# lnkloveating/MediQuery-RAG

Measured on AMD Instinct MI355X. Metric: queries/s (embed+top-k, k=5, b=256) over 1M×768 corpus; p50 single-query ms, higher is better.
Workload: dtype f32 (exact 3-way bf16 split, fp32 accumulate; exact fp32 top-k)

## Files before the change

include/mq.h:

```cpp
#ifndef MQ_H
#define MQ_H

#include <stdint.h>

#ifdef __cplusplus
extern "C" {
#endif

#define MQ_OK 0
#define MQ_EINVAL -1
#define MQ_ENOMEM -2
#define MQ_EHIP -3
#define MQ_EIO -4
#define MQ_ESTATE -5

#define MQ_DTYPE_F32 0
#define MQ_DTYPE_BF16 1
#define MQ_DTYPE_F32X6 2
#define MQ_DTYPE_F32_SCREEN 3

#define MQ_GELU_ERF 0
#define MQ_GELU_TANH 1
#define MQ_POOL_CLS 0
#define MQ_POOL_MEAN 1
// ... 10 lines not shown
int mq_device_count(void);

int mq_index_create(int device, int dim, int64_t capacity, int dtype, mq_index** out);
int mq_index_destroy(mq_index* ix);
int mq_index_size(const mq_index* ix, int64_t* n_rows);
int mq_index_dim(const mq_index* ix, int* dim);
int mq_index_add(mq_index* ix, const float* rows, int64_t n, int rows_on_device, void* stream);
int mq_index_reset(mq_index* ix);
int mq_index_search(mq_index* ix, const float* queries, int64_t nq, int k,
                    float* out_scores, int64_t* out_ids, int io_on_device, void* stream);
int mq_index_select(mq_index* src, const int64_t* rows, int64_t n, mq_index* dst);
int mq_index_get(mq_index* ix, int64_t row0, int64_t n, float* out, int out_on_device, void* stream);
int mq_index_set_precision(mq_index* ix, int dtype);
int mq_index_set_stream_threshold(mq_index* ix, int max_queries);
int mq_index_set_threshold_scan(mq_index* ix, int enabled);
int mq_index_set_int8_screen(mq_index* ix, int enabled);
int mq_index_set_async_screen(mq_index* ix, int enabled);
int mq_index_rescans(const mq_index* ix, int64_t* rescans, int64_t* remerges);
int mq_index_screen_fallbacks(const mq_index* ix, int64_t* to_direct, int64_t* to_split);
int mq_index_screen_skips(const mq_index* ix, int64_t* bf16_skips, int64_t* int8_skips);
int mq_index_data(mq_index* ix, void** device_rows);
int mq_index_set_timing(mq_index* ix, int enabled);
int mq_index_read_timing(mq_index* ix, float* ms, int n);
#define MQ_MASK_SET 0
#define MQ_MASK_AND 1
#define MQ_MASK_OR 2
#define MQ_MASK_CLEAR 3
int mq_mask_eval(const int32_t* codes, int64_t n, const uint8_t* lut, int n_lut, uint32_t* bits, int mode,
                 void* stream);
int mq_mask_eval_bits(const int32_t* codes, int64_t n, const uint64_t* lut_words, int n_lut, uint32_t* bits,
// ... 200 lines not shown
```

mediquery-rag_amd/csrc/index.hip:

```cpp
#include <algorithm>
#include <cmath>
#include <cstring>
#include <limits>
#include <memory>
#include <vector>

#include <unistd.h>

#include "common.hpp"
#include "gemm_f32.hpp"
#include "thresh.hpp"
#include "topk.hpp"

namespace mq {

__global__ __launch_bounds__(256) void add_rows_kernel(const float* __restrict__ src,
                                                       float* __restrict__ dst, int64_t n,
                                                       int dim) {
  const int lane = threadIdx.x & 63;
  const int64_t row = (int64_t)blockIdx.x * 4 + (threadIdx.x >> 6);
  if (row >= n) return;
  const floatx4* s = reinterpret_cast<const floatx4*>(src + row * dim);
  floatx4* d = reinterpret_cast<floatx4*>(dst + row * dim);
  const int nv = dim >> 2;
// ... 741 lines not shown
  }
  __syncthreads();
  MQ_FIN_TS(6);
  if (tid == 0) {
    const bool cert = ranked && nlive_sh <= kFinLive &&
                      (nl >= k ? tau[q] + e_sh < ek_sh : tau[q] == -INFINITY);
    if (!cert) fail[atomicAdd(n_fail, 1)] = q;
#if MQ_FIN_DBG & 16
    printf("FIN cnt %d nl %d dt %llu %llu %llu %llu %llu %llu\n", cnt, nl, tsx[1] - tsx[0], tsx[2] - tsx[1],
           tsx[3] - tsx[2], tsx[4] - tsx[3], tsx[5] - tsx[4], tsx[6] - tsx[5]);
#endif
  }
#undef MQ_FIN_TS
}

template <int KC, typename IdIn>
__device__ __forceinline__ void merge_threadlists(const float* __restrict__ cs,
                                                  const IdIn* __restrict__ ci, int n_lists,
                                                  int64_t nq, int k_in, int k_out,
                                                  float* __restrict__ out_s,
                                                  int64_t* __restrict__ out_i, int list_kc,
                                                  int* __restrict__ overflow, int64_t q) {
  constexpr int U = 8;
  __shared__ float ws[4 * MQ_MAX_K];
  __shared__ long long wi[4 * MQ_MAX_K];
  __shared__ float kth_s;
  __shared__ long long kth_i;
  const int tid = threadIdx.x, lane = tid & 63, wave = tid >> 6;
  float ls[KC];
  long long li[KC];
// ... 285 lines not shown
  } else {
    const ScanGeom g = scan_geom(nf, SearchNarrow::BM, SearchNarrow::BN, per_cu, num_cus, n_rows);
    if ((int)blockIdx.x >= g.G * g.nqt) return;
    flat_search_block<SearchNarrow, KC>(lds, Qc, nf, C, n_rows, dim, g.G, g.nqt, kl, cand_s, cand_i, blockIdx.x);
  }
}

template <int KC, int SCAN_KC>
__global__ __launch_bounds__(256) void fallback_merge_kernel(const float* __restrict__ cs,
                                                             const int* __restrict__ ci, int num_cus,
                                                             int64_t n_rows, int k, int kl,
                                                             const int* __restrict__ n_fail,
                                                             const int64_t* __restrict__ fail,
                                                             float* __restrict__ os,
                                                             int64_t* __restrict__ oi,
                                                             unsigned long long* __restrict__ total) {
  const int nf = __builtin_amdgcn_readfirstlane(*n_fail);
  const int64_t j = blockIdx.x;
  if (j == 0 && threadIdx.x == 0 && nf > 0) atomicAdd(total, (unsigned long long)nf);
  if (j >= nf) return;
  constexpr int per_cu = SCAN_KC <= 16 ? 2 : 1;
  int n_lists;
  if (nf > kFbNarrowMax) {
    const ScanGeom g = scan_geom(nf, SearchWide::BM, SearchWide::BN, per_cu, num_cus, n_rows);
    n_lists = g.G * SearchWide::WAVES_N * SearchSmem<SearchWide>::LPQ;
  } else {
    const ScanGeom g = scan_geom(nf, SearchNarrow::BM, SearchNarrow::BN, per_cu, num_cus, n_rows);
    n_lists = g.G * SearchNarrow::WAVES_N * SearchSmem<SearchNarrow>::LPQ;
  }
  const int64_t shift = (fail[j] - j) * k;
  merge_select_block<KC, int>(cs, ci, n_lists, nf, kl, k, os + shift, oi + shift, kl, nullptr, j);
}

}
// ... 42 lines not shown
  DevBuf stage, cand_s, cand_i, out_s, out_i;
  DevBuf sel;
  DevBuf rows16;
  int64_t n16 = 0;
  DevBuf stats16;
  DevBuf q16, coarse_s, coarse_i;
  DevBuf fb_cs, fb_ci;
  DevBuf flag;
  DevBuf tier_fail[4], tier_q[4], tier_s[4], tier_i[4];
  int64_t rescans = 0;
  int64_t remerges = 0;
  int64_t screen_fallbacks = 0;
  int64_t screen_passdowns = 0;
  int stream_max_q = 4;
  bool thresh_scan = true;
  DevBuf ts_lmax, ts_tau, ts_count, ts_cs, ts_ci;
  DevBuf i8c_cs, i8c_ci, i8c_count;
  DevBuf msel, mblk;
  DevBuf mres_s, mres_i;
  PinBuf pin;
  DevBuf rows8, scale8, err8, stats8;
  int64_t n8 = 0;
  int64_t masked_gathers = 0;
  bool i8_screen = true;
  double i8_fail_avg = 0.0;
  int i8_skip = 0;
  int64_t i8_skips = 0;
  bool async_screen = true;
  int sync_left = 0;
  DevBuf afb_q, afb_cs, afb_ci, afb_total;
  unsigned long long* afb_host = nullptr;
  hipEvent_t afb_event = nullptr;
  unsigned long long afb_seen = 0;
  double bf_fail_avg = 0.0;
  int bf_skip = 0;
  int64_t bf_skips = 0;
  Timeline tl;
  int precision = MQ_DTYPE_F32;
  std::mutex mu;
};

namespace {

template <class T, int KC>
void launch_search(const mq_index* ix, const float* q, int nq, int k, int G, int nqt,
                   float* cs, int* ci, hipStream_t s) {
// ... 218 lines not shown
  if (rc) return rc;
  const int64_t qpairs = nq * ix->dim / 2;
  hipLaunchKernelGGL(to_bf16_kernel, dim3((unsigned)((qpairs + 255) / 256)), dim3(256), 0, s, q,
                     ix->q16.as<unsigned>(), qpairs);
  MQ_HIP(hipGetLastError());
  return MQ_OK;
}

bool thresh_ok(const mq_index* ix, int64_t nq) {
  const int nch = ix->dim / 64;
  return ix->thresh_scan && nq > 64 && ix->dim % 64 == 0 && (nch == 4 || nch == 8 || nch == 12) &&
         ix->n >= kTsMinRows && ix->n < (1ll << 31);
}

int thresh_topk(mq_index* ix, const float* q16, int64_t nq, int kc, float* os, int64_t* oi,
                hipStream_t s, int tau_rank, int* fail_count, int64_t* fail, const unsigned* mask = nullptr) {
  const size_t n_lists = 2 * (size_t)ix->num_cus;
  int rc = ix->ts_lmax.ensure(n_lists * nq * sizeof(float));
  if (!rc) rc = ix->ts_tau.ensure(nq * sizeof(float));
  if (!rc) rc = ix->ts_count.ensure(nq * sizeof(int));
  if (!rc) rc = ix->ts_cs.ensure((size_t)nq * kTsCap * sizeof(float));
  if (!rc) rc = ix->ts_ci.ensure((size_t)nq * kTsCap * sizeof(int));
  if (rc) return rc;
  ThreshArgs a{q16, (int)nq, ix->rows16.as<unsigned char>(), ix->n, ix->dim, ix->num_cus, kc,
               ix->ts_lmax.as<float>(), ix->ts_tau.as<float>(), ix->ts_count.as<int>(),
               ix->ts_cs.as<float>(), ix->ts_ci.as<int>(), os, oi, tau_rank, fail_count, fail, mask};
  if (ix->tl.used > 4096) ix->tl.drain();
  launch_thresh(a, s, &ix->tl);
  ix->tl.close(s);
  MQ_HIP(hipGetLastError());
  return MQ_OK;
}

int ensure_i8(mq_index* ix, hipStream_t s) {
  int rc = ix->rows8.ensure((size_t)(ix->cap + kI8PadRows) * ix->dim);
  if (!rc) rc = ix->scale8.ensure((size_t)(ix->cap + kI8PadRows) * sizeof(float));
  if (!rc) rc = ix->err8.ensure((size_t)(ix->cap + kI8PadRows) * sizeof(float));
  if (!rc) rc = ix->stats8.ensure(2 * sizeof(unsigned));
  if (rc) return rc;
  if (ix->n8 < ix->n) {
    if (ix->n8 == 0) MQ_HIP(hipMemsetAsync(ix->stats8.p, 0, 2 * sizeof(unsigned), s));
    launch_i8_shadow(ix->rows + ix->n8 * ix->dim, ix->n - ix->n8, ix->dim,
                     ix->rows8.as<unsigned>() + ix->n8 * ix->dim / 4, ix->scale8.as<float>() + ix->n8,
// ... 142 lines not shown
}

template <class T>
void fallback_extent(const mq_index* ix, int64_t nf_lo, int64_t nf_hi, int per_cu, int kl,
                     int64_t* grid, int64_t* cand) {
  for (int64_t nqt = (nf_lo + T::BM - 1) / T::BM; nqt * T::BM < nf_hi + T::BM; ++nqt) {
    const int64_t nf = std::min(nf_hi, nqt * T::BM);
    const ScanGeom g = scan_geom(nf, T::BM, T::BN, per_cu, ix->num_cus, ix->n);
    *grid = std::max<int64_t>(*grid, (int64_t)g.G * g.nqt);
    *cand = std::max<int64_t>(*cand, (int64_t)g.G * T::WAVES_N * SearchSmem<T>::LPQ * nf * kl);
  }
}

template <int KC>
void launch_fallback_scans(mq_index* ix, int64_t nq, int k, const int* nf, const int64_t* fail,
                           float* os, int64_t* oi, int64_t grid, hipStream_t s) {
  const float* qc = ix->afb_q.as<float>();
  float* cs = ix->afb_cs.as<float>();
  int* ci = ix->afb_ci.as<int>();
  hipLaunchKernelGGL((fallback_search_kernel<KC>), dim3((unsigned)grid), dim3(256), 0, s, qc, nf, ix->rows,
                     ix->n, ix->dim, ix->num_cus, k, cs, ci);
  auto* tot = ix->afb_total.as<unsigned long long>();
  const dim3 mgrid((unsigned)nq);
  if (k <= 8)
    hipLaunchKernelGGL((fallback_merge_kernel<8, KC>), mgrid, dim3(256), 0, s, cs, ci, ix->num_cus, ix->n, k, k,
                       nf, fail, os, oi, tot);
  else
    hipLaunchKernelGGL((fallback_merge_kernel<16, KC>), mgrid, dim3(256), 0, s, cs, ci, ix->num_cus, ix->n, k,
                       k, nf, fail, os, oi, tot);
}

constexpr size_t kFbMaxBytes = 256ull << 20;

struct FallbackPlan {
  bool ok = false;
  int64_t grid = 0;
};

int fallback_prepare(mq_index* ix, int64_t nq, int k, FallbackPlan* fp) {
  const int per_cu = 2;
  int64_t grid_n = 0, grid_w = 0, cand = 0;
  fallback_extent<SearchNarrow>(ix, 1, std::min<int64_t>(nq, kFbNarrowMax), per_cu, k, &grid_n, &cand);
  if (nq > kFbNarrowMax) fallback_extent<SearchWide>(ix, kFbNarrowMax + 1, nq, per_cu, k, &grid_w, &cand);
  fp->ok = false;
  if ((size_t)cand * (sizeof(float) + sizeof(int)) + (size_t)nq * ix->dim * sizeof(float) > kFbMaxBytes)
    return MQ_OK;
  int rc = ix->afb_q.ensure((size_t)nq * ix->dim * sizeof(float));
  if (!rc) rc = ix->afb_cs.ensure((size_t)cand * sizeof(float));
  if (!rc) rc = ix->afb_ci.ensure((size_t)cand * sizeof(int));
  if (!rc && !ix->afb_total.p) {
    rc = ix->afb_total.ensure(sizeof(unsigned long long));
    if (!rc) MQ_HIP(hipMemset(ix->afb_total.p, 0, sizeof(unsigned long long)));
  }
  if (rc) return rc;
  if (!ix->afb_host) {
    MQ_HIP(hipHostMalloc((void**)&ix->afb_host, sizeof(unsigned long long), hipHostMallocDefault));
    *ix->afb_host = 0;
  }
  if (!ix->afb_event) MQ_HIP(hipEventCreateWithFlags(&ix->afb_event, hipEventDisableTiming));
  fp->ok = true;
  fp->grid = std::max(grid_n, grid_w);
  return MQ_OK;
}

static_assert(kScreenMaxK <= 16, "fallback_search_kernel<KC> has KC = 8 or 16");
int launch_async_fallback(mq_index* ix, const FallbackPlan& fp, int64_t nq, int k, float* os, int64_t* oi,
                          const int64_t* fail, hipStream_t s) {
  const int* nf = ix->flag.as<int>();
  if (k <= 8)
    launch_fallback_scans<8>(ix, nq, k, nf, fail, os, oi, fp.grid, s);
  else
    launch_fallback_scans<16>(ix, nq, k, nf, fail, os, oi, fp.grid, s);
  MQ_HIP(hipGetLastError());
  MQ_HIP(hipMemcpyAsync(ix->afb_host, ix->afb_total.p, sizeof(unsigned long long), hipMemcpyDeviceToHost, s));
  MQ_HIP(hipEventRecord(ix->afb_event, s));
  return MQ_OK;
}

int search_screened(mq_index* ix, int tier, const float* q, int64_t nq, int k, float* os,
                    int64_t* oi, hipStream_t s) {
  const bool bf = tier == TIER_BF16_STREAM || tier == TIER_BF16;
  const int want = tier == TIER_BF16 || tier == TIER_I8 ? MQ_MAX_K
                   : tier == TIER_BF16_STREAM ? (k + 11 <= 16 ? 16 : std::min(std::max(32, k + 16), MQ_MAX_K))
                   : (k + 3 <= 8 ? 8 : k + 8);
  const int kc = (int)std::min<int64_t>(want, ix->n);
  int rc = bf ? ensure_shadow(ix, s) : MQ_OK;
  if (!rc && tier == TIER_BF16) rc = queries_to_bf16(ix, q, nq, s);
  if (!rc) rc = ix->coarse_s.ensure((size_t)nq * kc * sizeof(float));
  if (!rc) rc = ix->coarse_i.ensure((size_t)nq * kc * sizeof(int64_t));
  if (!rc) rc = ix->flag.ensure(sizeof(int));
  if (!rc) rc = ix->tier_fail[tier].ensure((size_t)nq * sizeof(int64_t));
  if (rc) return rc;
  int64_t* fail = ix->tier_fail[tier].as<int64_t>();
  if (tier == TIER_I8) {
    rc = i8_topk(ix, q, nq, kc, nullptr, nullptr, s, ix->flag.as<int>(), k);
    if (rc) return rc;
    hipLaunchKernelGGL(i8_finish_kernel, dim3((unsigned)nq), dim3(kFinT), 0, s, q, ix->rows, ix->dim,
                       ix->ts_cs.as<float>(), ix->ts_ci.as<int>(), ix->ts_count.as<int>(),
                       i8_lists(ix->num_cus), ix->ts_tau.as<float>(), k, ix->stats8.as<unsigned>(), ix->err8.as<float>(), os, oi, ix->flag.as<int>(), fail);
    ix->tl.close(s);
    MQ_HIP(hipGetLastError());
  } else {
    const int kind = tier == TIER_X6 ? SCAN_X6 : tier == TIER_BF16 ? SCAN_BF16 : SCAN_STREAM16;
    const float* qs = tier == TIER_BF16 ? ix->q16.as<float>() : q;
    rc = kind == SCAN_BF16 ? bf16_candidates(ix, qs, nq, kc, ix->coarse_s.as<float>(), ix->coarse_i.as<int64_t>(), s)
                           : scan_topk(ix, kind, qs, nq, kc, ix->coarse_s.as<float>(), ix->coarse_i.as<int64_t>(), s);
    if (rc) return rc;
    const int mode = tier == TIER_X6 ? VERIFY_X6 : tier == TIER_BF16 ? VERIFY_BF16_Q16 : VERIFY_BF16_Q32;
    const unsigned* stats = bf ? ix->stats16.as<unsigned>() : nullptr;
// ... 3 lines not shown
    if (kc >= ix->n) return MQ_OK;
    FallbackPlan fp;
    if (tier == TIER_BF16) {
      poll_async_fallbacks(ix);
      if (ix->async_screen && ix->sync_left == 0 && k <= kScreenMaxK) {
        rc = fallback_prepare(ix, nq, k, &fp);
        if (rc) return rc;
      }
      if (!fp.ok && ix->sync_left > 0) --ix->sync_left;
    }
    MQ_HIP(hipMemsetAsync(ix->flag.p, 0, sizeof(int), s));
    hipLaunchKernelGGL(screen_verify_kernel, dim3((unsigned)((nq + 3) / 4)), dim3(256), 0, s, q,
                       ix->dim, ix->coarse_s.as<float>(), kc, os, k, nq, mode, stats, ix->flag.as<int>(),
                       fail, fp.ok ? ix->afb_q.as<float>() : nullptr);
    MQ_HIP(hipGetLastError());
    if (fp.ok) return launch_async_fallback(ix, fp, nq, k, os, oi, fail, s);
  }
  int n_fail = 0;
  rc = read_flag(ix, ix->flag.as<int>(), s, &n_fail);
  if (rc) return rc;
  if (tier == TIER_I8) {
    ix->i8_fail_avg = 0.9 * ix->i8_fail_avg + 0.1 * (double)n_fail / (double)nq;
    if (ix->i8_fail_avg > 0.3) {
      ix->i8_skip = 256;
      ix->i8_fail_avg = 0.0;
    }
  } else if (tier == TIER_BF16) {
    ix->bf_fail_avg = 0.75 * ix->bf_fail_avg + 0.25 * (double)n_fail / (double)nq;
    if (ix->bf_fail_avg > kBfSkipShare) {
      ix->bf_skip = kBfSkipSearches;
      ix->bf_fail_avg = 0.0;
// ... 358 lines not shown
  if (!stream_ok(ix)) {
    for (int64_t j = 0; j < nq; ++j) {
      const int rc = search_masked(ix, q + j * ix->dim, k, bits, os + j * k, oi + j * k, s);
      if (rc) return rc;
    }
    return MQ_OK;
  }
  if (!(exact_kind && k <= kScreenMaxK && thresh_ok(ix, nq) && ix->dim <= 1024)) {
    const int rc = masked_stream(ix, q, nq, k, bits, os, oi, s);
    if (rc) return rc;
    MQ_HIP(hipStreamSynchronize(s));
    return MQ_OK;
  }
  const int kc = (int)std::min<int64_t>(MQ_MAX_K, ix->n);
  int rc = ensure_shadow(ix, s);
  if (!rc) rc = queries_to_bf16(ix, q, nq, s);
  if (!rc) rc = ix->coarse_s.ensure((size_t)nq * kc * sizeof(float));
  if (!rc) rc = ix->coarse_i.ensure((size_t)nq * kc * sizeof(int64_t));
  if (!rc) rc = ix->flag.ensure(sizeof(int));
  if (!rc) rc = ix->tier_fail[TIER_BF16].ensure((size_t)nq * sizeof(int64_t));
  if (rc) return rc;
  rc = thresh_topk(ix, ix->q16.as<float>(), nq, kc, ix->coarse_s.as<float>(), ix->coarse_i.as<int64_t>(), s,
                   kTsRank, nullptr, nullptr, bits);
  if (rc) return rc;
  const unsigned* stats = ix->stats16.as<unsigned>();
  hipLaunchKernelGGL(rerank_kernel, dim3((unsigned)nq), dim3(256), 0, s, q, ix->rows, ix->dim,
                     ix->coarse_i.as<int64_t>(), kc, k, os, oi, ix->coarse_s.as<float>(), VERIFY_BF16_Q16, stats);
  MQ_HIP(hipMemsetAsync(ix->flag.p, 0, sizeof(int), s));
  int64_t* fail = ix->tier_fail[TIER_BF16].as<int64_t>();
  hipLaunchKernelGGL(screen_verify_kernel, dim3((unsigned)((nq + 3) / 4)), dim3(256), 0, s, q, ix->dim,
                     ix->coarse_s.as<float>(), kc, os, k, nq, VERIFY_BF16_Q16, stats, ix->flag.as<int>(), fail,
                     nullptr);
  MQ_HIP(hipGetLastError());
  int n_fail = 0;
  rc = read_flag(ix, ix->flag.as<int>(), s, &n_fail);
  if (rc) return rc;
  if (n_fail > 0) {
    ix->masked_gathers += n_fail;
    rc = ix->tier_q[TIER_BF16].ensure((size_t)n_fail * ix->dim * sizeof(float));
    if (!rc) rc = ix->tier_s[TIER_BF16].ensure((size_t)n_fail * k * sizeof(float));
    if (!rc) rc = ix->tier_i[TIER_BF16].ensure((size_t)n_fail * k * sizeof(int64_t));
    if (rc) return rc;
    float* sq = ix->tier_q[TIER_BF16].as<float>();
    hipLaunchKernelGGL(gather_rows_kernel, dim3((unsigned)((n_fail + 3) / 4)), dim3(256), 0, s, q, fail,
                       (int64_t)n_fail, ix->dim, sq);
    MQ_HIP(hipGetLastError());
    rc = masked_stream(ix, sq, n_fail, k, bits, ix->tier_s[TIER_BF16].as<float>(),
                       ix->tier_i[TIER_BF16].as<int64_t>(), s);
// ... 213 lines not shown
  MQ_CHECK_ARG(max_queries >= 0 && max_queries <= 16, "stream threshold must be in [0, 16] (got %d)",
               max_queries);
  std::lock_guard<std::mutex> lk(ix->mu);
  ix->stream_max_q = max_queries;
  return MQ_OK;
}

int mq_index_set_threshold_scan(mq_index* ix, int enabled) {
  clear_error();
  MQ_CHECK_ARG(ix, "NULL index");
  std::lock_guard<std::mutex> lk(ix->mu);
  ix->thresh_scan = enabled != 0;
  return MQ_OK;
}

int mq_index_set_int8_screen(mq_index* ix, int enabled) {
  clear_error();
  MQ_CHECK_ARG(ix, "NULL index");
  std::lock_guard<std::mutex> lk(ix->mu);
  ix->i8_screen = enabled != 0;
  ix->i8_skip = 0;
  ix->i8_fail_avg = 0.0;
  return MQ_OK;
}

int mq_index_screen_fallbacks(const mq_index* cix, int64_t* to_direct, int64_t* to_split) {
  clear_error();
  MQ_CHECK_ARG(cix, "NULL argument");
  mq_index* ix = const_cast<mq_index*>(cix);
  hipEvent_t ev = nullptr;
// ... 246 lines not shown
```

mediquery-rag_amd/csrc/thresh.hip:

```cpp
#include "gemm_f32.hpp"

#ifndef MQ_TS_DBG
#define MQ_TS_DBG 0
#endif
#if MQ_TS_DBG != 0 && !defined(MQ_MEASUREMENT_BUILD)
#error "MQ_TS_DBG computes wrong results: only a measurement build (-DMQ_MEASUREMENT_BUILD) may set it"
#endif
#include "thresh.hpp"
#include "topk.hpp"

namespace mq {

constexpr int kTsWaves = 8;
#ifndef MQ_TS_DMAW
#define MQ_TS_DMAW 4
#endif
constexpr int kTsDmaWaves = MQ_TS_DMAW;
static_assert(kTsDmaWaves == 8 || kTsDmaWaves == 4 || kTsDmaWaves == 2 || kTsDmaWaves == 1, "DMA waves");
constexpr int kTsQ = kTsWaves * 32;
constexpr int kTsBufs = 3;
constexpr int kTsPeriod = 16;
#ifndef MQ_TS_BF_PERIOD
#define MQ_TS_BF_PERIOD 16
#endif
// ... 186 lines not shown
    if (qvalid) lmax[(int64_t)q * (2 * gridDim.x) + blockIdx.x * 2 + h] = mx;
  } else {
    for (int j = lane; j < min(n_surv, kTsWaveSurv); j += 64) {
      const Survivor v = surv[j];
      const int slot = atomicAdd(count + v.q, 1);
      if (slot < kTsCap) {
        cs[(int64_t)v.q * kTsCap + slot] = v.s;
        ci[(int64_t)v.q * kTsCap + slot] = v.row;
      }
    }
  }
}

__global__ __launch_bounds__(256) void bf16_tau_kernel(const float* __restrict__ lmax, int n_lists,
                                                       int nq, int rank, float* __restrict__ tau,
                                                       int* __restrict__ count) {
  const int lane = threadIdx.x & 63;
  const int q = blockIdx.x * 4 + (threadIdx.x >> 6);
  if (q >= nq) return;
  TopList<kTsRank> t;
  t.init();
  for (int l = lane; l < n_lists; l += 64) {
    const float x = lmax[(int64_t)q * n_lists + l];
    if (t.beats_tail(x, l)) t.insert(x, l);
  }
  float kth = -INFINITY;
  for (int r = 0; r < rank; ++r) {
    float bs = t.s[0];
    int bi = t.id[0], bt = lane;
#pragma unroll
    for (int off = 32; off > 0; off >>= 1) {
// ... 10 lines not shown
  }
  if (lane == 0) {
    tau[q] = kth;
    count[q] = 0;
  }
}

__global__ __launch_bounds__(256) void bf16_select_kernel(const float* __restrict__ cs,
                                                          const int* __restrict__ ci,
                                                          const int* __restrict__ count,
                                                          const float* __restrict__ tau, int kc,
                                                          float* __restrict__ out_s,
                                                          int64_t* __restrict__ out_i,
                                                          int* __restrict__ fail_count,
                                                          int64_t* __restrict__ fail) {
  __shared__ float ls[kTsCap], fs[kTsCap], ts[256];
  __shared__ int li[kTsCap], fi[kTsCap], ti[256];
  __shared__ float cut_s;
  __shared__ int cut_i, nf;
  const int64_t q = blockIdx.x;
  const int tid = threadIdx.x;
  const int total = count[q];
  if (fail && tid == 0 && (total > kTsCap || total < kc)) fail[atomicAdd(fail_count, 1)] = q;
  const int cnt = min(total, kTsCap);
  float bs = -INFINITY;
  int bi = -1;
  for (int i = tid; i < cnt; i += 256) {
    const float x = cs[q * kTsCap + i];
    const int xi = ci[q * kTsCap + i];
    ls[i] = x;
    li[i] = xi;
    if (bi == -1 || better(x, (unsigned)xi, bs, (unsigned)bi)) {
      bs = x;
      bi = xi;
    }
  }
  auto rank_out = [&](const float* rs, const int* ri, int m) __attribute__((always_inline)) {
    for (int i = tid; i < m; i += 256) {
      const float x = rs[i];
      const int xi = ri[i];
      int rank = 0;
      for (int j = 0; j < m; ++j) rank += better(rs[j], (unsigned)ri[j], x, (unsigned)xi) ? 1 : 0;
      if (rank < kc) {
        out_s[q * kc + rank] = rank == kc - 1 && total > kTsCap ? INFINITY : x;
        out_i[q * kc + rank] = xi;
      }
    }
  };
  if (cnt <= 256) {
    __syncthreads();
    rank_out(ls, li, cnt);
  } else {
    ts[tid] = bs;
    ti[tid] = bi;
    if (tid == 0) {
      cut_s = -INFINITY;
      cut_i = -1;
      nf = 0;
    }
    __syncthreads();
    int rank = 0;
    for (int j = 0; j < 256; ++j) rank += better(ts[j], (unsigned)ti[j], bs, (unsigned)bi) ? 1 : 0;
    if (rank == kc - 1) {
      cut_s = bs;
      cut_i = bi;
    }
    __syncthreads();
    const float Ts = cut_s;
    const unsigned Ti = (unsigned)cut_i;
    const int lane = tid & 63;
    for (int base = 0; base < cnt; base += 256) {
      const int i = base + tid;
      const bool keep = i < cnt && !better(Ts, Ti, ls[i], (unsigned)li[i]);
      const unsigned long long bal = __ballot(keep);
      int slot0 = 0;
      if (lane == 0 && bal) slot0 = atomicAdd(&nf, __popcll(bal));
      slot0 = __shfl(slot0, 0);
      if (keep) {
        const int slot = slot0 + __builtin_amdgcn_mbcnt_hi((unsigned)(bal >> 32), __builtin_amdgcn_mbcnt_lo((unsigned)bal, 0));
        fs[slot] = ls[i];
        fi[slot] = li[i];
      }
    }
    __syncthreads();
    rank_out(fs, fi, nf);
  }
  for (int i = cnt + tid; i < kc; i += 256) {
    out_s[q * kc + i] = tau[q];
    out_i[q * kc + i] = -1;
  }
}

template <int NCH, bool MASKED>
void launch_nch(const ThreshArgs& a, hipStream_t s, Timeline* tl) {
  const int gy = (a.nq + kTsQ - 1) / kTsQ;
  const int G = gy == 1 ? a.num_cus : std::max(8, a.num_cus / gy / 8 * 8);
  const int64_t n_blocks = (a.n + kTsRows - 1) / kTsRows;
  const uint4* qb = reinterpret_cast<const uint4*>(a.q16);
  tl->mark(s, 0);
  hipLaunchKernelGGL((bf16_thresh_kernel<NCH, TS_MAX, MASKED>), dim3(G, gy), dim3(512), 0, s, qb, a.nq, a.rows,
                     a.n, n_blocks, kTsBfPeriod, a.tau, a.lmax, a.count, a.cs, a.ci, a.mask);
  tl->mark(s, 1);
  hipLaunchKernelGGL(bf16_tau_kernel, dim3((a.nq + 3) / 4), dim3(256), 0, s, a.lmax, 2 * G, a.nq,
                     a.tau_rank, a.tau, a.count);
  tl->mark(s, 0);
  hipLaunchKernelGGL((bf16_thresh_kernel<NCH, TS_APPEND, MASKED>), dim3(G, gy), dim3(512), 0, s, qb, a.nq,
                     a.rows, a.n, n_blocks, 1, a.tau, a.lmax, a.count, a.cs, a.ci, a.mask);
  tl->mark(s, 1);
  hipLaunchKernelGGL(bf16_select_kernel, dim3(a.nq), dim3(256), 0, s, a.cs, a.ci, a.count, a.tau, a.kc,
                     a.out_s, a.out_i, a.fail_count, a.fail);
}

template <bool MASKED>
void launch_dim(const ThreshArgs& a, hipStream_t s, Timeline* tl) {
  switch (a.dim / 64) {
    case 4: launch_nch<4, MASKED>(a, s, tl); break;
    case 8: launch_nch<8, MASKED>(a, s, tl); break;
    default: launch_nch<12, MASKED>(a, s, tl); break;
  }
}

void launch_thresh(const ThreshArgs& a, hipStream_t s, Timeline* tl) {
  if (a.mask)
// ... 482 lines not shown
```

mediquery-rag_amd/csrc/thresh.hpp:

```cpp
#pragma once

#include "common.hpp"

namespace mq {

constexpr int kTsRows = 32;
constexpr int kTsCap = 4096;
constexpr int64_t kTsMinRows = 65536;
constexpr int kTsRank = 8;

struct ThreshArgs {
  const float* q16;
  int nq;
  const unsigned char* rows;
  int64_t n;
  int dim;
  int num_cus;
  int kc;
  float* lmax;
  float* tau;
  int* count;
  float* cs;
  int* ci;
  float* out_s;
  int64_t* out_i;
  int tau_rank;
  int* fail_count;
  int64_t* fail;
  const unsigned* mask = nullptr;
};

void launch_thresh(const ThreshArgs& a, hipStream_t s, Timeline* tl);
hipError_t launch_thresh_append(const ThreshArgs& a, hipStream_t s);

#ifndef MQ_I8_WG
#define MQ_I8_WG 3
#endif
constexpr int kI8WgPerCu = MQ_I8_WG;
constexpr int kI8MaxLists = 1024;
constexpr int kI8PadRows = 16;
constexpr int kI8Seg = 16;
struct ThreshI8Args {
  const float* q;
  int nq;
// ... 9 lines not shown
  int* ci;
  int* zero;
  const unsigned* stats = nullptr;
  int k = 0;
  const unsigned* mask = nullptr;
};
int i8_lists(int num_cus);
void launch_i8_compact(const float* cs, const int* ci, const int* count, int lists, int nq, float* out_cs,
                       int* out_ci, int* out_count, hipStream_t s);
void launch_thresh_i8(const ThreshI8Args& a, hipStream_t s, Timeline* tl);
void launch_select(const float* cs, const int* ci, const int* count, const float* tau, int nq, int kc,
                   float* out_s, int64_t* out_i, hipStream_t s);
void launch_i8_shadow(const float* rows, int64_t n, int dim, unsigned* r8, float* scale, float* err,
                      unsigned* stats, hipStream_t s);

}
```

mediquery-rag_amd/mediquery_hip/_lib.py:

```python
import ctypes
import hashlib
import os

try:
    import torch
except Exception:
    torch = None

LIB_PATH = os.environ.get("MQ_LIB_PATH") or os.path.join(os.path.dirname(os.path.abspath(__file__)),
                                                          "libmqhip.so")

MQ_OK = 0
MQ_DTYPE_F32, MQ_DTYPE_BF16, MQ_DTYPE_F32X6, MQ_DTYPE_F32_SCREEN = 0, 1, 2, 3
MQ_GELU_ERF, MQ_GELU_TANH = 0, 1
MQ_POOL_CLS, MQ_POOL_MEAN = 0, 1
MQ_MAX_K = 64
MQ_RANGE_MAX_HITS = 4096
MQ_HEAD_MAX_LABELS = 8
MQ_JOIN_AUTO, MQ_JOIN_EXACT, MQ_JOIN_SCREEN = 0, 1, 2
MQ_KMEANS_MAX_CLUSTERS = 256
MQ_MASK_SET, MQ_MASK_AND, MQ_MASK_OR, MQ_MASK_CLEAR = 0, 1, 2, 3
MQ_CONTAINS_MAX_BYTES = 256
MQ_CONTAINS_SPAN_BYTES = 16384
MQ_LEX_MAX_TERMS = 128
# ... 42 lines not shown
    "mq_build_source_hash": (ctypes.c_char_p, []),
    "mq_device_count": (_I, []),
    "mq_index_create": (_I, [_I, _I, _I64, _I, _PP]),
    "mq_index_destroy": (_I, [_P]),
    "mq_index_size": (_I, [_P, ctypes.POINTER(_I64)]),
    "mq_index_dim": (_I, [_P, ctypes.POINTER(_I)]),
    "mq_index_add": (_I, [_P, _P, _I64, _I, _P]),
    "mq_index_reset": (_I, [_P]),
    "mq_index_search": (_I, [_P, _P, _I64, _I, _P, _P, _I, _P]),
    "mq_index_get": (_I, [_P, _I64, _I64, _P, _I, _P]),
    "mq_index_select": (_I, [_P, _P, _I64, _P]),
    "mq_index_data": (_I, [_P, _PP]),
    "mq_index_set_precision": (_I, [_P, _I]),
    "mq_index_set_stream_threshold": (_I, [_P, _I]),
    "mq_index_set_threshold_scan": (_I, [_P, _I]),
    "mq_index_set_int8_screen": (_I, [_P, _I]),
    "mq_index_set_async_screen": (_I, [_P, _I]),
    "mq_index_rescans": (_I, [_P, _P, _P]),
    "mq_index_screen_fallbacks": (_I, [_P, _P, _P]),
    "mq_index_screen_skips": (_I, [_P, _P, _P]),
    "mq_index_set_timing": (_I, [_P, _I]),
    "mq_index_read_timing": (_I, [_P, _P, _I]),
    "mq_index_save": (_I, [_P, ctypes.c_char_p]),
    "mq_index_load": (_I, [_P, ctypes.c_char_p]),
    "mq_index_save_rows": (_I, [_P, ctypes.c_char_p, ctypes.c_int64, ctypes.c_int64]),
    "mq_index_load_append": (_I, [_P, ctypes.c_char_p]),
    "mq_mask_eval": (_I, [_P, _I64, _P, _I, _P, _I, _P]),
    "mq_mask_eval_bits": (_I, [_P, _I64, _P, _I, _P, _I, _P]),
    "mq_mask_combine": (_I, [_P, _P, _I64, _I, _P]),
    "mq_mask_contains": (_I, [_P, _I64, _P, _I64, _P, _I, _I, _P, _I, _P, _P]),
# ... 170 lines not shown
```

mediquery-rag_amd/mediquery_hip/native.py:

```python
import ctypes

import numpy as np

from . import _lib
from .config import BertConfig
from .weights import head_from_state_dict, state_dict_to_blob, synthetic_state_dict


class FlatIndex:

    def __init__(self, dim=768, capacity=0, device=0, dtype=_lib.MQ_DTYPE_F32):
        h = ctypes.c_void_p()
        _lib.call("mq_index_create", device, dim, capacity, dtype, ctypes.byref(h))
        self._h = h
        self.dim = dim
        self.device = device

    def close(self):
        h, self._h = getattr(self, "_h", None), None
        if h:
            try:
                _lib.lib().mq_index_destroy(h)
            except Exception:
                pass
# ... 44 lines not shown
    def data_ptr(self):
        p = ctypes.c_void_p()
        _lib.call("mq_index_data", self._h, ctypes.byref(p))
        return p.value

    STAGES = ("flat_search_kernel", "merge_kernel")

    def set_precision(self, dtype):
        _lib.call("mq_index_set_precision", self._h, dtype)

    def set_stream_threshold(self, max_queries):
        _lib.call("mq_index_set_stream_threshold", self._h, int(max_queries))

    def set_threshold_scan(self, enabled=True):
        _lib.call("mq_index_set_threshold_scan", self._h, int(bool(enabled)))

    def set_int8_screen(self, enabled=True):
        _lib.call("mq_index_set_int8_screen", self._h, int(bool(enabled)))

    def set_async_screen(self, enabled=True):
        _lib.call("mq_index_set_async_screen", self._h, int(bool(enabled)))

    @property
    def rescans(self):
        n = ctypes.c_int64()
        _lib.call("mq_index_rescans", self._h, ctypes.byref(n), None)
        return n.value

    @property
    def remerges(self):
# ... 708 lines not shown
```

Baseline: 39850.

## Fuse bf16 threshold select, fp32 rerank and verify into one finish kernel

Adds a bf16_finish_kernel that runs the threshold candidate selection, exact fp32 rerank of the surviving candidates, and the screen-bound verification/fail recording inside one block per query. It replaces the select, rerank, memset and verify launches and the coarse_s/coarse_i round trip through global memory. The flag zeroing moves into the tau kernel, and the async fallback writes its total straight to pinned host memory instead of issuing a separate memcpy. It also prunes candidates below a cut derived from the error bound before reranking. The cost is a larger per-block shared-memory footprint and more work serialized in a single kernel.

```diff
diff --git a/include/mq.h b/include/mq.h
--- a/include/mq.h
+++ b/include/mq.h
@@ -48,6 +48,7 @@
 int mq_index_set_precision(mq_index* ix, int dtype);
 int mq_index_set_stream_threshold(mq_index* ix, int max_queries);
 int mq_index_set_threshold_scan(mq_index* ix, int enabled);
+int mq_index_set_fused_finish(mq_index* ix, int enabled);
 int mq_index_set_int8_screen(mq_index* ix, int enabled);
 int mq_index_set_async_screen(mq_index* ix, int enabled);
 int mq_index_rescans(const mq_index* ix, int64_t* rescans, int64_t* remerges);
diff --git a/mediquery-rag_amd/csrc/index.hip b/mediquery-rag_amd/csrc/index.hip
--- a/mediquery-rag_amd/csrc/index.hip
+++ b/mediquery-rag_amd/csrc/index.hip
@@ -779,6 +779,94 @@
 #undef MQ_FIN_TS
 }
 
+__global__ __launch_bounds__(256) void bf16_finish_kernel(
+    const float* __restrict__ Q, const float* __restrict__ rows, int dim, const float* __restrict__ cs,
+    const int* __restrict__ ci, const int* __restrict__ count, const float* __restrict__ tau, int kc, int k,
+    const unsigned* __restrict__ stats, float* __restrict__ out_s, int64_t* __restrict__ out_i,
+    int* __restrict__ n_fail, int64_t* __restrict__ fail, float* __restrict__ compact) {
+  __shared__ float cand_s[MQ_MAX_K], sc[MQ_MAX_K], es[kScreenMaxK];
+  __shared__ long long cand_i[MQ_MAX_K], sid[MQ_MAX_K], eid[kScreenMaxK];
+  __shared__ float e_sh;
+  __shared__ int n_live, fail_slot;
+  const int64_t q = blockIdx.x;
+  const int tid = threadIdx.x, lane = tid & 63, wave = tid >> 6;
+  const floatx4* q4 = reinterpret_cast<const floatx4*>(Q + q * dim);
+  select_block(cs, ci, count[q], tau[q], kc, q, tid, [&](int slot, float x, int xi) {
+    cand_s[slot] = x;
+    cand_i[slot] = xi;
+  });
+  if (tid < kc) {
+    sc[tid] = -INFINITY;
+    sid[tid] = -1;
+  }
+  if (tid < k) {
+    es[tid] = -INFINITY;
+    eid[tid] = -1;
+  }
+  __syncthreads();
+  if (wave == 0) {
+    const float E = screen_bound(Q, dim, q, VERIFY_BF16_Q16, stats, lane);
+    int live = kc;
+    if (k < kc) {
+      const float cut = cand_s[k - 1] - 2.f * E;
+      const bool keep = lane < kc && !(cand_s[lane] < cut);
+      live = __popcll(__ballot(keep)) + (kc > 64 ? kc - 64 : 0);
+      live = max(live, k);
+    }
+    if (lane == 0) {
+      n_live = live;
+      e_sh = E;
+    }
+  }
+  __syncthreads();
+  const int kl = n_live;
+  constexpr int U = 8;
+  const int slot = rerank_slot(lane);
+  for (int c0 = wave * U; c0 < kl; c0 += 4 * U) {
+    long long id[U];
+#pragma unroll
+    for (int u = 0; u < U; ++u) id[u] = c0 + u < kl ? cand_i[c0 + u] : -1;
+    const float dot = rerank_dots8(q4, rows, dim, id, lane);
+    long long my_id = id[0];
+#pragma unroll
+    for (int u = 1; u < U; ++u) my_id = slot == u ? id[u] : my_id;
+    if ((lane & 7) == 0 && c0 + slot < kl) {
+      sc[c0 + slot] = my_id >= 0 ? dot : -INFINITY;
+      sid[c0 + slot] = my_id;
+    }
+  }
+  __syncthreads();
+  if (tid < kc && sid[tid] >= 0) {
+    int rank = 0;
+    for (int u = 0; u < kc; ++u) rank += better(sc[u], sid[u], sc[tid], sid[tid]) ? 1 : 0;
+    if (rank < k) {
+      es[rank] = sc[tid];
+      eid[rank] = sid[tid];
+    }
+  }
+  __syncthreads();
+  if (tid < k) {
+    out_s[q * k + tid] = es[tid];
+    out_i[q * k + tid] = eid[tid];
+  }
+  if (tid == 0) {
+    const float ckc = cand_s[kc - 1];
+    const bool failed = !(ckc + e_sh < es[k - 1]) && ckc != -INFINITY;
+    int fs = -1;
+    if (failed) {
+      fs = atomicAdd(n_fail, 1);
+      fail[fs] = q;
+    }
+    fail_slot = fs;
+  }
+  if (!compact) return;
+  __syncthreads();
+  const int fslot = fail_slot;
+  if (fslot < 0) return;
+  floatx4* dst = reinterpret_cast<floatx4*>(compact + (int64_t)fslot * dim);
+  for (int i = tid; i < (dim >> 2); i += 256) dst[i] = q4[i];
+}
+
 template <int KC, typename IdIn>
 __device__ __forceinline__ void merge_threadlists(const float* __restrict__ cs,
                                                   const IdIn* __restrict__ ci, int n_lists,
@@ -1094,10 +1182,14 @@
                                                              const int64_t* __restrict__ fail,
                                                              float* __restrict__ os,
                                                              int64_t* __restrict__ oi,
-                                                             unsigned long long* __restrict__ total) {
+                                                             unsigned long long* __restrict__ total,
+                                                             unsigned long long* __restrict__ host_total) {
   const int nf = __builtin_amdgcn_readfirstlane(*n_fail);
   const int64_t j = blockIdx.x;
-  if (j == 0 && threadIdx.x == 0 && nf > 0) atomicAdd(total, (unsigned long long)nf);
+  if (j == 0 && threadIdx.x == 0 && nf > 0) {
+    const unsigned long long now = atomicAdd(total, (unsigned long long)nf) + (unsigned long long)nf;
+    if (host_total) __hip_atomic_store(host_total, now, __ATOMIC_RELEASE, __HIP_MEMORY_SCOPE_SYSTEM);
+  }
   if (j >= nf) return;
   constexpr int per_cu = SCAN_KC <= 16 ? 2 : 1;
   int n_lists;
@@ -1170,6 +1262,7 @@
   int64_t screen_passdowns = 0;
   int stream_max_q = 4;
   bool thresh_scan = true;
+  bool fused_finish = true;
   DevBuf ts_lmax, ts_tau, ts_count, ts_cs, ts_ci;
   DevBuf i8c_cs, i8c_ci, i8c_count;
   DevBuf msel, mblk;
@@ -1186,6 +1279,7 @@
   int sync_left = 0;
   DevBuf afb_q, afb_cs, afb_ci, afb_total;
   unsigned long long* afb_host = nullptr;
+  unsigned long long* afb_host_dev = nullptr;
   hipEvent_t afb_event = nullptr;
   unsigned long long afb_seen = 0;
   double bf_fail_avg = 0.0;
@@ -1434,7 +1528,8 @@
 }
 
 int thresh_topk(mq_index* ix, const float* q16, int64_t nq, int kc, float* os, int64_t* oi,
-                hipStream_t s, int tau_rank, int* fail_count, int64_t* fail, const unsigned* mask = nullptr) {
+                hipStream_t s, int tau_rank, int* fail_count, int64_t* fail, const unsigned* mask = nullptr,
+                int* finish_flag = nullptr) {
   const size_t n_lists = 2 * (size_t)ix->num_cus;
   int rc = ix->ts_lmax.ensure(n_lists * nq * sizeof(float));
   if (!rc) rc = ix->ts_tau.ensure(nq * sizeof(float));
@@ -1445,8 +1540,23 @@
   ThreshArgs a{q16, (int)nq, ix->rows16.as<unsigned char>(), ix->n, ix->dim, ix->num_cus, kc,
                ix->ts_lmax.as<float>(), ix->ts_tau.as<float>(), ix->ts_count.as<int>(),
                ix->ts_cs.as<float>(), ix->ts_ci.as<int>(), os, oi, tau_rank, fail_count, fail, mask};
+  a.select = finish_flag == nullptr;
+  a.zero_flag = finish_flag;
   if (ix->tl.used > 4096) ix->tl.drain();
   launch_thresh(a, s, &ix->tl);
+  if (a.select) ix->tl.close(s);
+  MQ_HIP(hipGetLastError());
+  return MQ_OK;
+}
+
+int thresh_finish(mq_index* ix, const float* q, int64_t nq, int kc, int k, float* os, int64_t* oi, hipStream_t s,
+                  int64_t* fail, float* compact, const unsigned* mask) {
+  const int rc = thresh_topk(ix, ix->q16.as<float>(), nq, kc, nullptr, nullptr, s, kTsRank, nullptr, nullptr, mask,
+                             ix->flag.as<int>());
+  if (rc) return rc;
+  hipLaunchKernelGGL(bf16_finish_kernel, dim3((unsigned)nq), dim3(256), 0, s, q, ix->rows, ix->dim,
+                     ix->ts_cs.as<float>(), ix->ts_ci.as<int>(), ix->ts_count.as<int>(), ix->ts_tau.as<float>(), kc,
+                     k, ix->stats16.as<unsigned>(), os, oi, ix->flag.as<int>(), fail, compact);
   ix->tl.close(s);
   MQ_HIP(hipGetLastError());
   return MQ_OK;
@@ -1619,7 +1729,8 @@
 
 template <int KC>
 void launch_fallback_scans(mq_index* ix, int64_t nq, int k, const int* nf, const int64_t* fail,
-                           float* os, int64_t* oi, int64_t grid, hipStream_t s) {
+                           float* os, int64_t* oi, int64_t grid, hipStream_t s,
+                           unsigned long long* host_tot) {
   const float* qc = ix->afb_q.as<float>();
   float* cs = ix->afb_cs.as<float>();
   int* ci = ix->afb_ci.as<int>();
@@ -1629,10 +1740,10 @@
   const dim3 mgrid((unsigned)nq);
   if (k <= 8)
     hipLaunchKernelGGL((fallback_merge_kernel<8, KC>), mgrid, dim3(256), 0, s, cs, ci, ix->num_cus, ix->n, k, k,
-                       nf, fail, os, oi, tot);
+                       nf, fail, os, oi, tot, host_tot);
   else
     hipLaunchKernelGGL((fallback_merge_kernel<16, KC>), mgrid, dim3(256), 0, s, cs, ci, ix->num_cus, ix->n, k,
-                       k, nf, fail, os, oi, tot);
+                       k, nf, fail, os, oi, tot, host_tot);
 }
 
 constexpr size_t kFbMaxBytes = 256ull << 20;
@@ -1661,6 +1772,7 @@
   if (!ix->afb_host) {
     MQ_HIP(hipHostMalloc((void**)&ix->afb_host, sizeof(unsigned long long), hipHostMallocDefault));
     *ix->afb_host = 0;
+    MQ_HIP(hipHostGetDevicePointer((void**)&ix->afb_host_dev, ix->afb_host, 0));
   }
   if (!ix->afb_event) MQ_HIP(hipEventCreateWithFlags(&ix->afb_event, hipEventDisableTiming));
   fp->ok = true;
@@ -1670,14 +1782,16 @@
 
 static_assert(kScreenMaxK <= 16, "fallback_search_kernel<KC> has KC = 8 or 16");
 int launch_async_fallback(mq_index* ix, const FallbackPlan& fp, int64_t nq, int k, float* os, int64_t* oi,
-                          const int64_t* fail, hipStream_t s) {
+                          const int64_t* fail, hipStream_t s, bool direct_total) {
   const int* nf = ix->flag.as<int>();
+  unsigned long long* host_tot = direct_total ? ix->afb_host_dev : nullptr;
   if (k <= 8)
-    launch_fallback_scans<8>(ix, nq, k, nf, fail, os, oi, fp.grid, s);
+    launch_fallback_scans<8>(ix, nq, k, nf, fail, os, oi, fp.grid, s, host_tot);
   else
-    launch_fallback_scans<16>(ix, nq, k, nf, fail, os, oi, fp.grid, s);
+    launch_fallback_scans<16>(ix, nq, k, nf, fail, os, oi, fp.grid, s, host_tot);
   MQ_HIP(hipGetLastError());
-  MQ_HIP(hipMemcpyAsync(ix->afb_host, ix->afb_total.p, sizeof(unsigned long long), hipMemcpyDeviceToHost, s));
+  if (!direct_total)
+    MQ_HIP(hipMemcpyAsync(ix->afb_host, ix->afb_total.p, sizeof(unsigned long long), hipMemcpyDeviceToHost, s));
   MQ_HIP(hipEventRecord(ix->afb_event, s));
   return MQ_OK;
 }
@@ -1690,14 +1804,26 @@
                    : (k + 3 <= 8 ? 8 : k + 8);
   const int kc = (int)std::min<int64_t>(want, ix->n);
   int rc = bf ? ensure_shadow(ix, s) : MQ_OK;
+  const bool fused = tier == TIER_BF16 && ix->fused_finish && k <= kScreenMaxK && thresh_ok(ix, nq);
   if (!rc && tier == TIER_BF16) rc = queries_to_bf16(ix, q, nq, s);
-  if (!rc) rc = ix->coarse_s.ensure((size_t)nq * kc * sizeof(float));
-  if (!rc) rc = ix->coarse_i.ensure((size_t)nq * kc * sizeof(int64_t));
+  if (!rc && !fused) rc = ix->coarse_s.ensure((size_t)nq * kc * sizeof(float));
+  if (!rc && !fused) rc = ix->coarse_i.ensure((size_t)nq * kc * sizeof(int64_t));
   if (!rc) rc = ix->flag.ensure(sizeof(int));
   if (!rc) rc = ix->tier_fail[tier].ensure((size_t)nq * sizeof(int64_t));
   if (rc) return rc;
   int64_t* fail = ix->tier_fail[tier].as<int64_t>();
-  if (tier == TIER_I8) {
+  if (fused) {
+    FallbackPlan fp;
+    poll_async_fallbacks(ix);
+    if (ix->async_screen && ix->sync_left == 0) {
+      rc = fallback_prepare(ix, nq, k, &fp);
+      if (rc) return rc;
+    }
+    if (!fp.ok && ix->sync_left > 0) --ix->sync_left;
+    rc = thresh_finish(ix, q, nq, kc, k, os, oi, s, fail, fp.ok ? ix->afb_q.as<float>() : nullptr, nullptr);
+    if (rc) return rc;
+    if (fp.ok) return launch_async_fallback(ix, fp, nq, k, os, oi, fail, s, true);
+  } else if (tier == TIER_I8) {
     rc = i8_topk(ix, q, nq, kc, nullptr, nullptr, s, ix->flag.as<int>(), k);
     if (rc) return rc;
     hipLaunchKernelGGL(i8_finish_kernel, dim3((unsigned)nq), dim3(kFinT), 0, s, q, ix->rows, ix->dim,
@@ -1731,7 +1857,7 @@
                        ix->dim, ix->coarse_s.as<float>(), kc, os, k, nq, mode, stats, ix->flag.as<int>(),
                        fail, fp.ok ? ix->afb_q.as<float>() : nullptr);
     MQ_HIP(hipGetLastError());
-    if (fp.ok) return launch_async_fallback(ix, fp, nq, k, os, oi, fail, s);
+    if (fp.ok) return launch_async_fallback(ix, fp, nq, k, os, oi, fail, s, false);
   }
   int n_fail = 0;
   rc = read_flag(ix, ix->flag.as<int>(), s, &n_fail);
@@ -2120,24 +2246,30 @@
   }
   const int kc = (int)std::min<int64_t>(MQ_MAX_K, ix->n);
   int rc = ensure_shadow(ix, s);
+  const bool fused = ix->fused_finish;
   if (!rc) rc = queries_to_bf16(ix, q, nq, s);
-  if (!rc) rc = ix->coarse_s.ensure((size_t)nq * kc * sizeof(float));
-  if (!rc) rc = ix->coarse_i.ensure((size_t)nq * kc * sizeof(int64_t));
+  if (!rc && !fused) rc = ix->coarse_s.ensure((size_t)nq * kc * sizeof(float));
+  if (!rc && !fused) rc = ix->coarse_i.ensure((size_t)nq * kc * sizeof(int64_t));
   if (!rc) rc = ix->flag.ensure(sizeof(int));
   if (!rc) rc = ix->tier_fail[TIER_BF16].ensure((size_t)nq * sizeof(int64_t));
   if (rc) return rc;
-  rc = thresh_topk(ix, ix->q16.as<float>(), nq, kc, ix->coarse_s.as<float>(), ix->coarse_i.as<int64_t>(), s,
-                   kTsRank, nullptr, nullptr, bits);
-  if (rc) return rc;
-  const unsigned* stats = ix->stats16.as<unsigned>();
-  hipLaunchKernelGGL(rerank_kernel, dim3((unsigned)nq), dim3(256), 0, s, q, ix->rows, ix->dim,
-                     ix->coarse_i.as<int64_t>(), kc, k, os, oi, ix->coarse_s.as<float>(), VERIFY_BF16_Q16, stats);
-  MQ_HIP(hipMemsetAsync(ix->flag.p, 0, sizeof(int), s));
   int64_t* fail = ix->tier_fail[TIER_BF16].as<int64_t>();
-  hipLaunchKernelGGL(screen_verify_kernel, dim3((unsigned)((nq + 3) / 4)), dim3(256), 0, s, q, ix->dim,
-                     ix->coarse_s.as<float>(), kc, os, k, nq, VERIFY_BF16_Q16, stats, ix->flag.as<int>(), fail,
-                     nullptr);
-  MQ_HIP(hipGetLastError());
+  if (fused) {
+    rc = thresh_finish(ix, q, nq, kc, k, os, oi, s, fail, nullptr, bits);
+    if (rc) return rc;
+  } else {
+    rc = thresh_topk(ix, ix->q16.as<float>(), nq, kc, ix->coarse_s.as<float>(), ix->coarse_i.as<int64_t>(), s,
+                     kTsRank, nullptr, nullptr, bits);
+    if (rc) return rc;
+    const unsigned* stats = ix->stats16.as<unsigned>();
+    hipLaunchKernelGGL(rerank_kernel, dim3((unsigned)nq), dim3(256), 0, s, q, ix->rows, ix->dim,
+                       ix->coarse_i.as<int64_t>(), kc, k, os, oi, ix->coarse_s.as<float>(), VERIFY_BF16_Q16, stats);
+    MQ_HIP(hipMemsetAsync(ix->flag.p, 0, sizeof(int), s));
+    hipLaunchKernelGGL(screen_verify_kernel, dim3((unsigned)((nq + 3) / 4)), dim3(256), 0, s, q, ix->dim,
+                       ix->coarse_s.as<float>(), kc, os, k, nq, VERIFY_BF16_Q16, stats, ix->flag.as<int>(), fail,
+                       nullptr);
+    MQ_HIP(hipGetLastError());
+  }
   int n_fail = 0;
   rc = read_flag(ix, ix->flag.as<int>(), s, &n_fail);
   if (rc) return rc;
@@ -2381,6 +2513,14 @@
   return MQ_OK;
 }
 
+int mq_index_set_fused_finish(mq_index* ix, int enabled) {
+  clear_error();
+  MQ_CHECK_ARG(ix, "NULL index");
+  std::lock_guard<std::mutex> lk(ix->mu);
+  ix->fused_finish = enabled != 0;
+  return MQ_OK;
+}
+
 int mq_index_set_int8_screen(mq_index* ix, int enabled) {
   clear_error();
   MQ_CHECK_ARG(ix, "NULL index");
diff --git a/mediquery-rag_amd/csrc/thresh.hip b/mediquery-rag_amd/csrc/thresh.hip
--- a/mediquery-rag_amd/csrc/thresh.hip
+++ b/mediquery-rag_amd/csrc/thresh.hip
@@ -224,7 +224,9 @@
 
 __global__ __launch_bounds__(256) void bf16_tau_kernel(const float* __restrict__ lmax, int n_lists,
                                                        int nq, int rank, float* __restrict__ tau,
-                                                       int* __restrict__ count) {
+                                                       int* __restrict__ count,
+                                                       int* __restrict__ zero_flag) {
+  if (zero_flag && blockIdx.x == 0 && threadIdx.x == 0) *zero_flag = 0;
   const int lane = threadIdx.x & 63;
   const int q = blockIdx.x * 4 + (threadIdx.x >> 6);
   if (q >= nq) return;
@@ -265,81 +267,14 @@
                                                           int64_t* __restrict__ out_i,
                                                           int* __restrict__ fail_count,
                                                           int64_t* __restrict__ fail) {
-  __shared__ float ls[kTsCap], fs[kTsCap], ts[256];
-  __shared__ int li[kTsCap], fi[kTsCap], ti[256];
-  __shared__ float cut_s;
-  __shared__ int cut_i, nf;
   const int64_t q = blockIdx.x;
   const int tid = threadIdx.x;
   const int total = count[q];
   if (fail && tid == 0 && (total > kTsCap || total < kc)) fail[atomicAdd(fail_count, 1)] = q;
-  const int cnt = min(total, kTsCap);
-  float bs = -INFINITY;
-  int bi = -1;
-  for (int i = tid; i < cnt; i += 256) {
-    const float x = cs[q * kTsCap + i];
-    const int xi = ci[q * kTsCap + i];
-    ls[i] = x;
-    li[i] = xi;
-    if (bi == -1 || better(x, (unsigned)xi, bs, (unsigned)bi)) {
-      bs = x;
-      bi = xi;
-    }
-  }
-  auto rank_out = [&](const float* rs, const int* ri, int m) __attribute__((always_inline)) {
-    for (int i = tid; i < m; i += 256) {
-      const float x = rs[i];
-      const int xi = ri[i];
-      int rank = 0;
-      for (int j = 0; j < m; ++j) rank += better(rs[j], (unsigned)ri[j], x, (unsigned)xi) ? 1 : 0;
-      if (rank < kc) {
-        out_s[q * kc + rank] = rank == kc - 1 && total > kTsCap ? INFINITY : x;
-        out_i[q * kc + rank] = xi;
-      }
-    }
-  };
-  if (cnt <= 256) {
-    __syncthreads();
-    rank_out(ls, li, cnt);
-  } else {
-    ts[tid] = bs;
-    ti[tid] = bi;
-    if (tid == 0) {
-      cut_s = -INFINITY;
-      cut_i = -1;
-      nf = 0;
-    }
-    __syncthreads();
-    int rank = 0;
-    for (int j = 0; j < 256; ++j) rank += better(ts[j], (unsigned)ti[j], bs, (unsigned)bi) ? 1 : 0;
-    if (rank == kc - 1) {
-      cut_s = bs;
-      cut_i = bi;
-    }
-    __syncthreads();
-    const float Ts = cut_s;
-    const unsigned Ti = (unsigned)cut_i;
-    const int lane = tid & 63;
-    for (int base = 0; base < cnt; base += 256) {
-      const int i = base + tid;
-      const bool keep = i < cnt && !better(Ts, Ti, ls[i], (unsigned)li[i]);
-      const unsigned long long bal = __ballot(keep);
-      int slot0 = 0;
-      if (lane == 0 && bal) slot0 = atomicAdd(&nf, __popcll(bal));
-      slot0 = __shfl(slot0, 0);
-      if (keep) {
-        const int slot = slot0 + __builtin_amdgcn_mbcnt_hi((unsigned)(bal >> 32), __builtin_amdgcn_mbcnt_lo((unsigned)bal, 0));
-        fs[slot] = ls[i];
-        fi[slot] = li[i];
-      }
-    }
-    __syncthreads();
-    rank_out(fs, fi, nf);
-  }
-  for (int i = cnt + tid; i < kc; i += 256) {
-    out_s[q * kc + i] = tau[q];
-    out_i[q * kc + i] = -1;
-  }
+  select_block(cs, ci, total, tau[q], kc, q, tid, [&](int slot, float x, int xi) {
+    out_s[q * kc + slot] = x;
+    out_i[q * kc + slot] = xi;
+  });
 }
 
 template <int NCH, bool MASKED>
@@ -353,11 +288,12 @@
                      a.n, n_blocks, kTsBfPeriod, a.tau, a.lmax, a.count, a.cs, a.ci, a.mask);
   tl->mark(s, 1);
   hipLaunchKernelGGL(bf16_tau_kernel, dim3((a.nq + 3) / 4), dim3(256), 0, s, a.lmax, 2 * G, a.nq,
-                     a.tau_rank, a.tau, a.count);
+                     a.tau_rank, a.tau, a.count, a.zero_flag);
   tl->mark(s, 0);
   hipLaunchKernelGGL((bf16_thresh_kernel<NCH, TS_APPEND, MASKED>), dim3(G, gy), dim3(512), 0, s, qb, a.nq,
                      a.rows, a.n, n_blocks, 1, a.tau, a.lmax, a.count, a.cs, a.ci, a.mask);
   tl->mark(s, 1);
+  if (!a.select) return;
   hipLaunchKernelGGL(bf16_select_kernel, dim3(a.nq), dim3(256), 0, s, a.cs, a.ci, a.count, a.tau, a.kc,
                      a.out_s, a.out_i, a.fail_count, a.fail);
 }
diff --git a/mediquery-rag_amd/csrc/thresh.hpp b/mediquery-rag_amd/csrc/thresh.hpp
--- a/mediquery-rag_amd/csrc/thresh.hpp
+++ b/mediquery-rag_amd/csrc/thresh.hpp
@@ -28,6 +28,8 @@
   int* fail_count;
   int64_t* fail;
   const unsigned* mask = nullptr;
+  bool select = true;
+  int* zero_flag = nullptr;
 };
 
 void launch_thresh(const ThreshArgs& a, hipStream_t s, Timeline* tl);
@@ -67,4 +69,74 @@
 void launch_i8_shadow(const float* rows, int64_t n, int dim, unsigned* r8, float* scale, float* err,
                       unsigned* stats, hipStream_t s);
 
+template <class Put>
+__device__ __forceinline__ void select_block(const float* __restrict__ cs, const int* __restrict__ ci, int total,
+                                             float tau_q, int kc, int64_t q, int tid, Put put) {
+  __shared__ float ls[kTsCap], fs[kTsCap], ts[256];
+  __shared__ int li[kTsCap], fi[kTsCap], ti[256];
+  __shared__ float cut_s;
+  __shared__ int cut_i, nf;
+  const int cnt = min(total, kTsCap);
+  float bs = -INFINITY;
+  int bi = -1;
+  for (int i = tid; i < cnt; i += 256) {
+    const float x = cs[q * kTsCap + i];
+    const int xi = ci[q * kTsCap + i];
+    ls[i] = x;
+    li[i] = xi;
+    if (bi == -1 || better(x, (unsigned)xi, bs, (unsigned)bi)) {
+      bs = x;
+      bi = xi;
+    }
+  }
+  auto rank_out = [&](const float* rs, const int* ri, int m) __attribute__((always_inline)) {
+    for (int i = tid; i < m; i += 256) {
+      const float x = rs[i];
+      const int xi = ri[i];
+      int rank = 0;
+      for (int j = 0; j < m; ++j) rank += better(rs[j], (unsigned)ri[j], x, (unsigned)xi) ? 1 : 0;
+      if (rank < kc) put(rank, rank == kc - 1 && total > kTsCap ? INFINITY : x, xi);
+    }
+  };
+  if (cnt <= 256) {
+    __syncthreads();
+    rank_out(ls, li, cnt);
+  } else {
+    ts[tid] = bs;
+    ti[tid] = bi;
+    if (tid == 0) {
+      cut_s = -INFINITY;
+      cut_i = -1;
+      nf = 0;
+    }
+    __syncthreads();
+    int rank = 0;
+    for (int j = 0; j < 256; ++j) rank += better(ts[j], (unsigned)ti[j], bs, (unsigned)bi) ? 1 : 0;
+    if (rank == kc - 1) {
+      cut_s = bs;
+      cut_i = bi;
+    }
+    __syncthreads();
+    const float Ts = cut_s;
+    const unsigned Ti = (unsigned)cut_i;
+    const int lane = tid & 63;
+    for (int base = 0; base < cnt; base += 256) {
+      const int i = base + tid;
+      const bool keep = i < cnt && !better(Ts, Ti, ls[i], (unsigned)li[i]);
+      const unsigned long long bal = __ballot(keep);
+      int slot0 = 0;
+      if (lane == 0 && bal) slot0 = atomicAdd(&nf, __popcll(bal));
+      slot0 = __shfl(slot0, 0);
+      if (keep) {
+        const int slot = slot0 + __builtin_amdgcn_mbcnt_hi((unsigned)(bal >> 32), __builtin_amdgcn_mbcnt_lo((unsigned)bal, 0));
+        fs[slot] = ls[i];
+        fi[slot] = li[i];
+      }
+    }
+    __syncthreads();
+    rank_out(fs, fi, nf);
+  }
+  for (int i = cnt + tid; i < kc; i += 256) put(i, tau_q, -1);
 }
+
+}
diff --git a/mediquery-rag_amd/mediquery_hip/_lib.py b/mediquery-rag_amd/mediquery_hip/_lib.py
--- a/mediquery-rag_amd/mediquery_hip/_lib.py
+++ b/mediquery-rag_amd/mediquery_hip/_lib.py
@@ -80,6 +80,7 @@
     "mq_index_set_precision": (_I, [_P, _I]),
     "mq_index_set_stream_threshold": (_I, [_P, _I]),
     "mq_index_set_threshold_scan": (_I, [_P, _I]),
+    "mq_index_set_fused_finish": (_I, [_P, _I]),
     "mq_index_set_int8_screen": (_I, [_P, _I]),
     "mq_index_set_async_screen": (_I, [_P, _I]),
     "mq_index_rescans": (_I, [_P, _P, _P]),
diff --git a/mediquery-rag_amd/mediquery_hip/native.py b/mediquery-rag_amd/mediquery_hip/native.py
--- a/mediquery-rag_amd/mediquery_hip/native.py
+++ b/mediquery-rag_amd/mediquery_hip/native.py
@@ -82,6 +82,9 @@
 
     def set_threshold_scan(self, enabled=True):
         _lib.call("mq_index_set_threshold_scan", self._h, int(bool(enabled)))
+
+    def set_fused_finish(self, enabled=True):
+        _lib.call("mq_index_set_fused_finish", self._h, int(bool(enabled)))
 
     def set_int8_screen(self, enabled=True):
         _lib.call("mq_index_set_int8_screen", self._h, int(bool(enabled)))
```

After: 39900, median of 6. About the same (+0.1%).
